# XiSHEN0220/RANSAC-Flow

Measured on AMD Instinct MI355X. Metric: aligned image-pairs/sec @480×640, 1/2/4/8 MI355X; max-abs flow Δ vs ref, higher is better.
Workload: dtype f32

## Files before the change

include/rfx_api.h:

```cpp
#ifndef RFX_API_H
#define RFX_API_H

#include <stddef.h>
#include <stdint.h>

#ifdef __cplusplus
extern "C" {
#endif

#define RFX_OK 0
#define RFX_E_ARG (-1)
#define RFX_E_LIMIT (-2)

#define RFX_ACT_NONE 0
#define RFX_ACT_RELU 1
#define RFX_ACT_SIGMOID 2

const char* rfx_version(void);

#define RFX_ABI_VERSION 12
int rfx_abi_version(void);

int rfx_group_begin(void);
int rfx_group_end(void* stream);
int rfx_group_abort(void);
int rfx_group_side_streams(int enable);

int rfx_conv2d_f32(const float* in, const float* wT, const int32_t* ktab, const float* scale,
                   const float* shift, const float* residual, float* out, int N, int Cin, int Hin,
                   int Win, int Cout, int KH, int KW, int stride, int pad, int act, void* stream);

int rfx_conv2d_tile_variant(int N, int Cout, int Hout, int Wout);

int rfx_conv2d_kernel_id(int N, int Cin, int Cout, int KH, int KW, int stride, int pad, int Hout, int Wout);

int rfx_conv3x3_f32(const float* in, const float* wP, const float* scale, const float* shift, const float* residual,
                    float* out, int N, int Cin, int H, int W, int Cout, int act, int k_chunk, void* stream);
int rfx_conv3x3_kernel_id(int N, int Cin, int Cout, int H, int W, int k_chunk);
int rfx_conv3x3_s2_f32(const float* in, const float* wP, const float* scale, const float* shift, const float* residual,
                       float* out, int N, int Cin, int H, int W, int Cout, int act, void* stream);

int rfx_conv3x3_conv1x1_kernel_id(int N, int H, int W, int Cmid);
int rfx_conv3x3_conv1x1_f32(const float* in, const float* wP2, const float* scale2, const float* shift2, int act2,
                            const float* wQ3, const float* scale3, const float* shift3, const float* residual, int act3,
                            float* out, int N, int Cin, int H, int W, int Cmid, int Cexp, void* stream);

int rfx_maxpool2d_f32(const float* in, float* out, int NC, int Hin, int Win, int k, int stride,
                      int pad, void* stream);

int rfx_blurpool2d_f32(const float* in, float* out, int NC, int Hin, int Win, int stride, void* stream);

int rfx_maxblurpool2d_f32(const float* in, float* out, int NC, int Hin, int Win, int stride, void* stream);

int rfx_stem_conv3x3_maxblur_f32(const float* in, const float* wT, const float* scale, const float* shift, float* out,
                                 int N, int H, int W, int Cout, void* stream);

int rfx_stem_conv7x7_maxpool_f32(const float* in, const float* wT, const float* scale, const float* shift, float* out,
                                 int N, int H, int W, int Cout, void* stream);

int rfx_l2norm_nchw_f32(const float* in, float* out, int N, int C, int HW, long long out_batch_stride,
                        long long out_chan_stride, void* stream);
int rfx_l2norm_nchw_scatter_f32(const float* in, float* out, int N, int C, int HW, const long long* dst_off,
                                long long out_chan_stride, void* stream);

int rfx_flow_head_f32(const float* logits, float* flow, int N, int K, int rows, int cols, void* stream);

int rfx_resize_bilinear_f32(const float* in, float* out, int NC, int Hin, int Win, int Hout, int Wout,
                            int align_corners, void* stream);

int rfx_lanczos_pass_u8(const uint8_t* in, uint8_t* out, int N, int inH, int inW, int outH, int outW, int C,
                        const int32_t* bounds, const int32_t* weights, int ksize, int vertical, int row_offset,
                        void* stream);

int rfx_u8_to_f32_chw(const uint8_t* in, float* raw, float* norm, int N, int H, int W, const float* mean3_host,
                      const float* std3_host, void* stream);

int rfx_copy_cols_f32(const float* src, float* dst, long long rows, int w_src, int w_dst, void* stream);

int rfx_corr_neigh_f32(const float* x, const float* y, float* out, int N, int C, int H, int W, int K,
                       void* stream);
int rfx_corr_neigh_variant_f32(const float* x, const float* y, float* out, int N, int C, int H, int W, int K,
                               int variant, void* stream);

int rfx_corr_neigh_bidir_f32(const float* x, const float* y, float* out_xy, float* out_yx, int N, int C, int H, int W, int K,
                             void* stream);
int rfx_corr_timing(int enable);
int rfx_corr_timing_collect(float* us_out, int cap);

int rfx_warp_grid_f32(const float* Hm, float* grid, int B, int h, int w, void* stream);

int rfx_grid_sample_f32(const float* in, const float* grid, float* out, int N, int C, int Hi, int Wi,
                        int Ho, int Wo, int align_corners, void* stream);

int rfx_compose_flow_f32(const float* flowDown, const float* coarseGrid, float* flow12, float* inb,
                         float* flowUp, int N, int hd, int wd, int Hc, int Wc, int H, int W, int clamp, void* stream);

int rfx_flow_grad_clamp_f32(const float* flowCoarse, const float* grid, float* flowGrad, float* flow, int B, int H, int W,
                            int grid_batch, void* stream);

int rfx_merge_multi_h_f32(const float* flow, const float* match12, long long match12_stride, const float* cyc,
                          const float* inb, int n, long long HW, float th, int multiH, float* flowGlobal,
                          float* matchGlobal, uint8_t* binary, void* stream);

int rfx_match_score_f32(const float* match12, long long match12_stride, const float* cyc, const float* inb, int n,
                        long long HW, float* score, void* stream);

size_t rfx_remove_small_cc_ws_bytes(int N, int H, int W);
int rfx_remove_small_cc_f32(const float* in, float* out, int N, int H, int W, float match_th, int max_area, void* ws,
                            void* stream);

size_t rfx_mutual_nn_ws_bytes(int nA, int nB);
int rfx_mutual_nn_f32(const float* featA, int ldA, int nA, const float* featB, int ldB, int nB, int C,
                      const float* maskB, int64_t* idx1, int64_t* idx2, int32_t* count, void* ws, int score_chunk,
                      void* stream);

int rfx_mutual_nn_batched_f32(const float* featA, int ldA, int nA, long long strideA, const float* featB, int ldB,
                              int nB, long long strideB, int C, const float* maskB, int64_t* idx1, int64_t* idx2,
                              int32_t* count, void* ws, int batch, int score_chunk, void* stream);

int rfx_mutual_nn_ragged_f32(const float* featA, int ldA, const float* featB, int ldB, const int32_t* nA, const int32_t* nB,
                             int maxNA, int maxNB, int C, const float* maskB, int64_t* idx1, int64_t* idx2, int cap,
                             int32_t* count, void* ws, int batch, int score_chunk, void* stream);

int rfx_dlt4_homography(const float* X, const float* Y, int N, float* Hout, void* stream);

int rfx_prediction_f32(const float* match1, const float* match2, int n, const float* Hs, int N, float* err,
                       void* stream);

int rfx_score_hypotheses(const float* match1, const float* match2, int n, const int64_t* samples, int N,
                         float tol, float* Hout, int64_t* counts, uint8_t* flags_out, void* ws, void* stream);

size_t rfx_ransac_ws_bytes(int n, int N);
int rfx_ransac_h4(const float* match1, const float* match2, int n, const int64_t* samples, int N,
                  float tol, float* bestH, uint8_t* inlier, int32_t* result, void* ws, void* stream);

size_t rfx_ransac_batched_ws_bytes(int cap, int N, int batch);
int rfx_ransac_h4_batched(const float* match1, const float* match2, const int32_t* n, int cap, const int64_t* samples,
                          int N, float tol, float* bestH, uint8_t* inlier, int32_t* result, void* ws, int batch,
                          void* stream);

int rfx_ransac_h4_batched_stage(const float* match1, const float* match2, const int32_t* n, int cap, const int64_t* samples,
                                int N, float tol, float* bestH, uint8_t* inlier, int32_t* result, void* ws, int batch,
                                int stages, void* stream);
int rfx_ransac_degenerate_list(const void* ws, int cap, int N, int batch, int32_t* idx, int32_t* count, int kcap, void* stream);
int rfx_ransac_patch_h(void* ws, int cap, int N, int batch, const int32_t* idx, const int32_t* count, const float* Hpatch,
                       int kcap, void* stream);
int rfx_ransac_degenerate_gather(const void* ws, const float* match1, const float* match2, const int32_t* n, int cap,
                                 const int64_t* samples, int N, int batch, int32_t* idx, int32_t* count, int32_t* off,
                                 int32_t* off_host, float* xy_rows, int row_cap, void* stream);
int rfx_ransac_patch_h_rows(void* ws, int cap, int N, int batch, const int32_t* idx, const int32_t* count, const int32_t* off,
                            const float* H_rows, int row_cap, void* stream);
int rfx_dlt4_homography_flags(const float* X, const float* Y, int N, float* Hout, uint8_t* flags, void* stream);

int rfx_gather_matches_f32(const int64_t* idx1, const int64_t* idx2, const int32_t* n, int cap, const float* xa,
                           const float* ya, const float* xb, const float* yb, float* match1, float* match2, int batch,
                           void* stream);

int rfx_gather_matches_ragged_f32(const int64_t* idx1, const int64_t* idx2, const int32_t* n, int cap, const float* xa,
                                  const float* ya, const long long* offA, const float* xb, const float* yb, const long long* offB,
                                  float* match1, float* match2, int batch, void* stream);

int rfx_draw_samples_i64(const int32_t* n, int64_t* samples, int N, int batch, uint64_t seed, uint64_t stream_id,
                         const int32_t* pair_ids, void* stream);

int rfx_keep_mask_f32(const float* mask, const float* bg, const int32_t* active, int n_active, int h, int w, int rt, int ct,
                      float* keep, void* stream);

int rfx_filter_matches_f32(const int64_t* idx1, const int64_t* idx2, const int32_t* count, int cap, const int32_t* active,
                           int n_active, const float* mask, const float* bg, int h, int w, int rt, int ct, const float* xa,
                           const float* ya, const float* xb, const float* yb, float* match1, float* match2, int32_t* n_out,
                           int32_t* kept, void* stream);

size_t rfx_multih_accept_ws_bytes(int n_active);
int rfx_multih_accept_f32(const float* match, float* mask, const float* bg, const int32_t* active, int n_active, int h, int w,
                          const int32_t* ransac_result, const int32_t* n_match, int32_t* nbH, double th, int mode,
                          int32_t* accept, float* gain, void* ws, const float* bestH, const float* flowDown8,
                          const float* match12Down8, const float* match21Down8, int h8, int w8, const float* flowD2, int hd2,
                          int wd2, float* rec, long long rec_stride, int max_h, int off_H, int off_flow, int off_match,
                          int off_d2, void* stream);

int rfx_filter_matches_ragged_f32(const int64_t* idx1, const int64_t* idx2, const int32_t* count, int cap, const int32_t* active,
                                  int n_active, const float* mask, const float* bg, const long long* moff, const int32_t* geom,
                                  const float* xa, const float* ya, const long long* offA, const float* xb, const float* yb,
                                  const long long* offB, float* match1, float* match2, int32_t* n_out, int32_t* kept,
                                  void* stream);

size_t rfx_multih_accept_ragged_ws_bytes(int n_active);
int rfx_multih_accept_ragged_f32(const float* match, const long long* match_off, float* mask, const float* bg,
                                 const long long* moff, const int32_t* geom, const int32_t* active, int n_active, long long max_hw,
                                 const int32_t* ransac_result, const int32_t* n_match, int32_t* nbH, double th, int mode,
                                 int32_t* accept, float* gain, void* ws, const float* bestH, const float* flowDown8,
                                 const float* match12Down8, const float* match21Down8, const long long* off8, float* rec,
                                 long long rec_stride, int max_h, int off_H, int off_flow, void* stream);

int rfx_conv1x1_split_f32(const float* in, const void* wS, const float* scale, const float* shift, const float* residual,
                          float* out, int N, int Cin, int HW, int Cout, int act, void* stream);
int rfx_conv1x1_split_strided_f32(const float* in, const void* wS, const float* scale, const float* shift, const float* residual,
                                  float* out, int N, int Cin, int Hin, int Win, int Cout, int stride, int act, void* stream);
int rfx_conv3x3_split_f32(const float* in, const void* wS3, const float* scale, const float* shift, const float* residual,
                          float* out, int N, int Cin, int H, int W, int Cout, int act, void* stream);
int rfx_conv3x3_split_s2_f32(const float* in, const void* wS3, const float* scale, const float* shift, const float* residual,
                             float* out, int N, int Cin, int H, int W, int Cout, int act, void* stream);

int rfx_conv2d_dilated_f32(const float* in, const float* wT, const int32_t* ktab, const float* scale,
                           const float* shift, const float* residual, float* out, int N, int Cin, int Hin,
                           int Win, int Cout, int KH, int KW, int stride, int pad, int dilation, int act, void* stream);
int rfx_adaptive_avgpool2d_f32(const float* in, float* out, int NC, int Hin, int Win, int Hout, int Wout, void* stream);
int rfx_softmax_accum_f32(const float* logits, float* scores, int N, int C, long long HW, float div, int accumulate, void* stream);
int rfx_argmax_mask_f32(const float* scores, int N, int C, long long HW, int id, int complement, float* mask, int32_t* pred,
                        void* stream);

#ifdef __cplusplus
}
#endif
#endif
```

ransac-flow_amd/csrc/conv1x1s.hip:

```cpp
#include "common.h"
#include "conv_epilogue.h"
#include "group.h"

namespace {

typedef __bf16 bf16x8 __attribute__((ext_vector_type(8)));
typedef __bf16 bf16x2 __attribute__((ext_vector_type(2)));
typedef float f32x2 __attribute__((ext_vector_type(2)));
typedef unsigned u32x4 __attribute__((ext_vector_type(4)));

struct C1SArgs {
    const float* in; const u32x4* wS; const float* scale; const float* shift; const float* res; float* out;
    int Cin, HW, Cout, act, Mpad;
    long long P;
    int tilesM, tilesP;
    int stride, Win, Wo, HWin;
};

__device__ __forceinline__ unsigned pack_bf16(float a, float b) {
    const f32x2 v = {a, b};
    const bf16x2 h = __builtin_convertvector(v, bf16x2);
    unsigned u;
    __builtin_memcpy(&u, &h, 4);
    return u;
}
__device__ __forceinline__ void split_pair(float a, float b, unsigned& hi, unsigned& mid, unsigned& lo) {
    hi = pack_bf16(a, b);
    const float ra = a - __uint_as_float(hi << 16), rb = b - __uint_as_float(hi & 0xffff0000u);
    mid = pack_bf16(ra, rb);
    lo = pack_bf16(ra - __uint_as_float(mid << 16), rb - __uint_as_float(mid & 0xffff0000u));
}
__device__ __forceinline__ bf16x8 as_frag(const u32x4& w) {
    bf16x8 f;
    __builtin_memcpy(&f, &w, 16);
    return f;
}

template <int TM>
__device__ __forceinline__ void conv1x1_split_body(const C1SArgs& a, const unsigned bx) {
    constexpr int BM = 64 * TM, BN = 128, KB = 16;
    constexpr int A_WORDS = 3 * 2 * BM;
    constexpr int NA = (A_WORDS + 255) / 256;
    __shared__ u32x4 As[2][3][2][BM];
    __shared__ u32x4 Bs[2][3][2][BN];
    __shared__ float s_scale[BM], s_shift[BM];

    const int t = threadIdx.x, lane = t & 63, wave = t >> 6;
    const int wm = wave >> 1, wn = wave & 1;
    const int lrow = lane >> 5, lcol = lane & 31;
    const size_t HW = (size_t)a.HW, HWin = (size_t)a.HWin;
    const int nwg = a.tilesM * a.tilesP;
    const int nk = a.Cin / KB;

    int m0; long long n0;
    {
        const int v = (int)bx, q = nwg / 8, r = nwg % 8, xcd = v % 8, j = v / 8;
        const int bid = (xcd < r ? xcd * (q + 1) : r * (q + 1) + (xcd - r) * q) + j;
        m0 = (bid % a.tilesM) * BM;
        n0 = (long long)(bid / a.tilesM) * BN;
    }
    constexpr int A_ROWS = 256 / BM;
    const u32x4* wsrc = a.wS + (size_t)(t / BM) * a.Mpad + m0 + t % BM;
    auto a_on = [&](int j) { return (j + 1) * 256 <= A_WORDS || t + 256 * j < A_WORDS; };
    const int bh = t >> 7, bp = t & 127;
    const float* bsrc;
    {
        long long p = n0 + bp;
        if (p >= a.P) p = a.P - 1;
        const long long n = p / a.HW;
        int off = (int)(p - n * a.HW);
        if (a.stride != 1) { const int y = off / a.Wo, x = off - y * a.Wo; off = y * a.stride * a.Win + x * a.stride; }
        bsrc = a.in + ((size_t)n * a.Cin + 8 * bh) * HWin + (size_t)off;
    }
    u32x4 ra[NA];
    float rb[8];
    auto load_stage = [&](int kb) {
#pragma unroll
        for (int j = 0; j < NA; ++j)
            ra[j] = wsrc[((size_t)kb * 6 + (a_on(j) ? A_ROWS * j : 0)) * a.Mpad];
#pragma unroll
        for (int i = 0; i < 8; ++i) rb[i] = bsrc[(size_t)(kb * KB + i) * HWin];
    };
    auto store_stage = [&](int buf) {
#pragma unroll
        for (int j = 0; j < NA; ++j)
            if (a_on(j)) (&As[buf][0][0][0])[t + 256 * j] = ra[j];
        u32x4 hi, mid, lo;
#pragma unroll
        for (int i = 0; i < 4; ++i) {
            unsigned h_, m_, l_;
            split_pair(rb[2 * i], rb[2 * i + 1], h_, m_, l_);
            hi[i] = h_; mid[i] = m_; lo[i] = l_;
        }
        Bs[buf][0][bh][bp] = hi;
        Bs[buf][1][bh][bp] = mid;
        Bs[buf][2][bh][bp] = lo;
    };
    if (t < BM) {
        const int m = m0 + t;
        s_scale[t] = (a.scale && m < a.Cout) ? a.scale[m] : 1.0f;
        s_shift[t] = (a.shift && m < a.Cout) ? a.shift[m] : 0.0f;
    }
    load_stage(0);
    store_stage(0);
    if (nk > 1) load_stage(1);
    __syncthreads();

    f32x16 acc[TM][2], low[TM][2];
#pragma unroll
    for (int i = 0; i < TM; ++i)
#pragma unroll
        for (int j = 0; j < 2; ++j)
#pragma unroll
            for (int r = 0; r < 16; ++r) { acc[i][j][r] = 0.0f; low[i][j][r] = 0.0f; }

    for (int s = 0; s < nk; ++s) {
        const int cur = s & 1;
        bf16x8 af[3][TM], bf[3][2];
#pragma unroll
        for (int pc = 0; pc < 3; ++pc) {
#pragma unroll
            for (int i = 0; i < TM; ++i) af[pc][i] = as_frag(As[cur][pc][lrow][wm * TM * 32 + i * 32 + lcol]);
#pragma unroll
            for (int j = 0; j < 2; ++j) bf[pc][j] = as_frag(Bs[cur][pc][lrow][wn * 64 + j * 32 + lcol]);
        }
        if (s + 1 < nk) store_stage(cur ^ 1);
        if (s + 2 < nk) load_stage(s + 2);
        __builtin_amdgcn_sched_barrier(0);
#pragma unroll
        for (int i = 0; i < TM; ++i)
#pragma unroll
            for (int j = 0; j < 2; ++j) {
                low[i][j] = __builtin_amdgcn_mfma_f32_32x32x16_bf16(af[2][i], bf[0][j], low[i][j], 0, 0, 0);
                low[i][j] = __builtin_amdgcn_mfma_f32_32x32x16_bf16(af[0][i], bf[2][j], low[i][j], 0, 0, 0);
                low[i][j] = __builtin_amdgcn_mfma_f32_32x32x16_bf16(af[1][i], bf[1][j], low[i][j], 0, 0, 0);
            }
#pragma unroll
        for (int i = 0; i < TM; ++i)
#pragma unroll
            for (int j = 0; j < 2; ++j) {
                low[i][j] = __builtin_amdgcn_mfma_f32_32x32x16_bf16(af[1][i], bf[0][j], low[i][j], 0, 0, 0);
                low[i][j] = __builtin_amdgcn_mfma_f32_32x32x16_bf16(af[0][i], bf[1][j], low[i][j], 0, 0, 0);
                acc[i][j] = __builtin_amdgcn_mfma_f32_32x32x16_bf16(af[0][i], bf[0][j], acc[i][j], 0, 0, 0);
            }
        __builtin_amdgcn_sched_barrier(0);
        __syncthreads();
    }
#pragma unroll
    for (int i = 0; i < TM; ++i)
#pragma unroll
        for (int j = 0; j < 2; ++j)
#pragma unroll
            for (int r = 0; r < 16; ++r) acc[i][j][r] += low[i][j][r];

    size_t pix_off[2];
    bool pix_ok[2];
#pragma unroll
    for (int j = 0; j < 2; ++j) {
        long long pp = n0 + wn * 64 + j * 32 + lcol;
        pix_ok[j] = pp < a.P;
        if (!pix_ok[j]) pp = a.P - 1;
        const long long n = pp / a.HW;
        pix_off[j] = (size_t)n * a.Cout * HW + (size_t)(pp - n * a.HW);
    }
    conv_epilogue<TM, 2, false>(acc, s_scale, s_shift, a.res, a.out, a.act, a.Cout, HW, m0, wm, lrow, pix_off, pix_ok, m0 + BM <= a.Cout);
}

template <int TM>
__global__ __launch_bounds__(256, 2) void conv1x1_split_kernel(C1SArgs a) {
    conv1x1_split_body<TM>(a, blockIdx.x);
}

template <int TM>
__global__ __launch_bounds__(256, 2) void conv1x1_split_group_kernel(RfxGroupArgs<C1SArgs> g) {
    const unsigned y = blockIdx.y;
    if (blockIdx.x >= g.gx[y]) return;
    conv1x1_split_body<TM>(g.p[y], blockIdx.x);
}

template <int TM>
static int c1s_group_launch(const void* blob, const unsigned* gx, int n, hipStream_t st) {
    return rfx_group_launch_impl<C1SArgs>(conv1x1_split_group_kernel<TM>, 256, blob, gx, n, st);
}

template <int TM>
int launch_split(C1SArgs& a, hipStream_t st) {
    a.tilesM = (a.Cout + 64 * TM - 1) / (64 * TM);
    a.tilesP = (int)((a.P + 127) / 128);
    const long long nwg = (long long)a.tilesM * a.tilesP;
    if (nwg > 0x7fffffffLL) return RFX_E_LIMIT;
    if (rfx_group_recording()) return rfx_group_record(&c1s_group_launch<TM>, &a, sizeof(a), (unsigned)nwg);
    hipLaunchKernelGGL((conv1x1_split_kernel<TM>), dim3((unsigned)nwg), dim3(256), 0, st, a);
    RFX_LAUNCH_CHECK();
    return RFX_OK;
}

}

static int conv1x1_split_launch(const float* in, const void* wS, const float* scale, const float* shift, const float* residual,
                                float* out, int N, int Cin, int Hin, int Win, int Cout, int stride, int act, void* stream) {
    if (!in || !wS || !out || N <= 0 || Cin <= 0 || Hin <= 0 || Win <= 0 || Cout <= 0) return RFX_E_ARG;
    if (Cin % 16 != 0 || (stride != 1 && stride != 2)) return RFX_E_ARG;
    if (act != RFX_ACT_NONE && act != RFX_ACT_RELU && act != RFX_ACT_SIGMOID) return RFX_E_ARG;
    const int Ho = (Hin - 1) / stride + 1, Wo = (Win - 1) / stride + 1;
    C1SArgs a;
    a.in = in; a.wS = reinterpret_cast<const u32x4*>(wS); a.scale = scale; a.shift = shift; a.res = residual; a.out = out;
    a.Cin = Cin; a.HW = Ho * Wo; a.Cout = Cout; a.act = act; a.Mpad = (Cout + 127) / 128 * 128;
    a.P = (long long)N * a.HW;
    a.stride = stride; a.Win = Win; a.Wo = Wo; a.HWin = Hin * Win;
    return Cout > 64 ? launch_split<2>(a, rfx_stream(stream)) : launch_split<1>(a, rfx_stream(stream));
}

extern "C" int rfx_conv1x1_split_f32(const float* in, const void* wS, const float* scale, const float* shift, const float* residual,
                                     float* out, int N, int Cin, int HW, int Cout, int act, void* stream) {
    return conv1x1_split_launch(in, wS, scale, shift, residual, out, N, Cin, 1, HW, Cout, 1, act, stream);
}

extern "C" int rfx_conv1x1_split_strided_f32(const float* in, const void* wS, const float* scale, const float* shift, const float* residual,
                                             float* out, int N, int Cin, int Hin, int Win, int Cout, int stride, int act, void* stream) {
    return conv1x1_split_launch(in, wS, scale, shift, residual, out, N, Cin, Hin, Win, Cout, stride, act, stream);
}
```

ransac-flow_amd/rfx/_lib.py:

```python
import ctypes
import os
from ctypes import c_int, c_int32, c_int64, c_uint64, c_float, c_double, c_void_p, c_size_t, c_longlong, c_char_p

_HERE = os.path.dirname(os.path.abspath(__file__))
LIB_PATH = os.environ.get("RFX_LIB") or os.path.normpath(os.path.join(_HERE, "..", "librfx.so"))

SIGNATURES = {
    "rfx_version": (c_char_p, []),
    "rfx_abi_version": (c_int, []),
    "rfx_group_begin": (c_int, []),
    "rfx_group_end": (c_int, [c_void_p]),
    "rfx_group_abort": (c_int, []),
    "rfx_group_side_streams": (c_int, [c_int]),
    "rfx_conv2d_f32": (c_int, [c_void_p] * 7 + [c_int] * 10 + [c_void_p]),
    "rfx_conv2d_dilated_f32": (c_int, [c_void_p] * 7 + [c_int] * 11 + [c_void_p]),
    "rfx_conv1x1_split_f32": (c_int, [c_void_p] * 6 + [c_int] * 5 + [c_void_p]),
    "rfx_conv3x3_split_f32": (c_int, [c_void_p] * 6 + [c_int] * 6 + [c_void_p]),
    "rfx_conv3x3_split_s2_f32": (c_int, [c_void_p] * 6 + [c_int] * 6 + [c_void_p]),
    "rfx_conv1x1_split_strided_f32": (c_int, [c_void_p] * 6 + [c_int] * 7 + [c_void_p]),
    "rfx_adaptive_avgpool2d_f32": (c_int, [c_void_p, c_void_p] + [c_int] * 5 + [c_void_p]),
    "rfx_softmax_accum_f32": (c_int, [c_void_p, c_void_p, c_int, c_int, c_longlong, c_float, c_int, c_void_p]),
    "rfx_argmax_mask_f32": (c_int, [c_void_p, c_int, c_int, c_longlong, c_int, c_int, c_void_p, c_void_p, c_void_p]),
    "rfx_conv2d_tile_variant": (c_int, [c_int] * 4),
    "rfx_conv2d_kernel_id": (c_int, [c_int] * 9),
    "rfx_conv3x3_f32": (c_int, [c_void_p] * 6 + [c_int] * 7 + [c_void_p]),
    "rfx_conv3x3_kernel_id": (c_int, [c_int] * 6),
    "rfx_conv3x3_s2_f32": (c_int, [c_void_p] * 6 + [c_int] * 6 + [c_void_p]),
    "rfx_conv3x3_conv1x1_kernel_id": (c_int, [c_int] * 4),
    "rfx_conv3x3_conv1x1_f32": (c_int, [c_void_p] * 4 + [c_int] + [c_void_p] * 4 + [c_int, c_void_p] + [c_int] * 6 + [c_void_p]),
    "rfx_maxpool2d_f32": (c_int, [c_void_p, c_void_p] + [c_int] * 6 + [c_void_p]),
    "rfx_blurpool2d_f32": (c_int, [c_void_p, c_void_p] + [c_int] * 4 + [c_void_p]),
    "rfx_maxblurpool2d_f32": (c_int, [c_void_p, c_void_p] + [c_int] * 4 + [c_void_p]),
    "rfx_stem_conv3x3_maxblur_f32": (c_int, [c_void_p] * 5 + [c_int] * 4 + [c_void_p]),
    "rfx_stem_conv7x7_maxpool_f32": (c_int, [c_void_p] * 5 + [c_int] * 4 + [c_void_p]),
    "rfx_l2norm_nchw_f32": (c_int, [c_void_p, c_void_p, c_int, c_int, c_int, c_longlong, c_longlong, c_void_p]),
    "rfx_l2norm_nchw_scatter_f32": (c_int, [c_void_p, c_void_p, c_int, c_int, c_int, c_void_p, c_longlong, c_void_p]),
    "rfx_flow_head_f32": (c_int, [c_void_p, c_void_p] + [c_int] * 4 + [c_void_p]),
    "rfx_resize_bilinear_f32": (c_int, [c_void_p, c_void_p] + [c_int] * 6 + [c_void_p]),
    "rfx_lanczos_pass_u8": (c_int, [c_void_p, c_void_p] + [c_int] * 6 + [c_void_p, c_void_p] + [c_int] * 3 + [c_void_p]),
    "rfx_u8_to_f32_chw": (c_int, [c_void_p] * 3 + [c_int] * 3 + [c_void_p] * 3),
    "rfx_copy_cols_f32": (c_int, [c_void_p, c_void_p, c_longlong, c_int, c_int, c_void_p]),
    "rfx_corr_neigh_f32": (c_int, [c_void_p] * 3 + [c_int] * 5 + [c_void_p]),
    "rfx_corr_neigh_variant_f32": (c_int, [c_void_p] * 3 + [c_int] * 6 + [c_void_p]),
    "rfx_corr_neigh_bidir_f32": (c_int, [c_void_p] * 4 + [c_int] * 5 + [c_void_p]),
    "rfx_corr_timing": (c_int, [c_int]),
    "rfx_corr_timing_collect": (c_int, [c_void_p, c_int]),
    "rfx_warp_grid_f32": (c_int, [c_void_p, c_void_p] + [c_int] * 3 + [c_void_p]),
    "rfx_grid_sample_f32": (c_int, [c_void_p] * 3 + [c_int] * 7 + [c_void_p]),
    "rfx_compose_flow_f32": (c_int, [c_void_p] * 5 + [c_int] * 8 + [c_void_p]),
    "rfx_flow_grad_clamp_f32": (c_int, [c_void_p] * 4 + [c_int] * 4 + [c_void_p]),
    "rfx_merge_multi_h_f32": (c_int, [c_void_p, c_void_p, c_longlong, c_void_p, c_void_p, c_int, c_longlong, c_float, c_int,
                                      c_void_p, c_void_p, c_void_p, c_void_p]),
    "rfx_match_score_f32": (c_int, [c_void_p, c_longlong, c_void_p, c_void_p, c_int, c_longlong, c_void_p, c_void_p]),
    "rfx_remove_small_cc_ws_bytes": (c_size_t, [c_int] * 3),
    "rfx_remove_small_cc_f32": (c_int, [c_void_p, c_void_p, c_int, c_int, c_int, c_float, c_int, c_void_p, c_void_p]),
    "rfx_mutual_nn_ws_bytes": (c_size_t, [c_int, c_int]),
    "rfx_mutual_nn_f32": (c_int, [c_void_p, c_int, c_int, c_void_p, c_int, c_int, c_int] + [c_void_p] * 5 + [c_int, c_void_p]),
    "rfx_mutual_nn_batched_f32": (c_int, [c_void_p, c_int, c_int, c_longlong, c_void_p, c_int, c_int, c_longlong, c_int]
                                  + [c_void_p] * 5 + [c_int, c_int, c_void_p]),
    "rfx_mutual_nn_ragged_f32": (c_int, [c_void_p, c_int, c_void_p, c_int, c_void_p, c_void_p, c_int, c_int, c_int, c_void_p,
                                         c_void_p, c_void_p, c_int, c_void_p, c_void_p, c_int, c_int, c_void_p]),
    "rfx_dlt4_homography": (c_int, [c_void_p, c_void_p, c_int, c_void_p, c_void_p]),
    "rfx_prediction_f32": (c_int, [c_void_p, c_void_p, c_int, c_void_p, c_int, c_void_p, c_void_p]),
    "rfx_score_hypotheses": (c_int, [c_void_p, c_void_p, c_int, c_void_p, c_int, c_float] + [c_void_p] * 5),
    "rfx_ransac_ws_bytes": (c_size_t, [c_int, c_int]),
    "rfx_ransac_h4": (c_int, [c_void_p, c_void_p, c_int, c_void_p, c_int, c_float] + [c_void_p] * 5),
    "rfx_ransac_batched_ws_bytes": (c_size_t, [c_int, c_int, c_int]),
    "rfx_ransac_h4_batched_stage": (c_int, [c_void_p, c_void_p, c_void_p, c_int, c_void_p, c_int, c_float] + [c_void_p] * 4
                                    + [c_int, c_int, c_void_p]),
    "rfx_ransac_degenerate_list": (c_int, [c_void_p, c_int, c_int, c_int, c_void_p, c_void_p, c_int, c_void_p]),
    "rfx_ransac_patch_h": (c_int, [c_void_p, c_int, c_int, c_int, c_void_p, c_void_p, c_void_p, c_int, c_void_p]),
    "rfx_ransac_degenerate_gather": (c_int, [c_void_p] * 4 + [c_int, c_void_p, c_int, c_int] + [c_void_p] * 5 + [c_int, c_void_p]),
    "rfx_ransac_patch_h_rows": (c_int, [c_void_p, c_int, c_int, c_int] + [c_void_p] * 4 + [c_int, c_void_p]),
    "rfx_dlt4_homography_flags": (c_int, [c_void_p, c_void_p, c_int, c_void_p, c_void_p, c_void_p]),
    "rfx_ransac_h4_batched": (c_int, [c_void_p, c_void_p, c_void_p, c_int, c_void_p, c_int, c_float] + [c_void_p] * 4
                              + [c_int, c_void_p]),
    "rfx_gather_matches_f32": (c_int, [c_void_p, c_void_p, c_void_p, c_int] + [c_void_p] * 6 + [c_int, c_void_p]),
    "rfx_gather_matches_ragged_f32": (c_int, [c_void_p, c_void_p, c_void_p, c_int] + [c_void_p] * 8 + [c_int, c_void_p]),
    "rfx_draw_samples_i64": (c_int, [c_void_p, c_void_p, c_int, c_int, c_uint64, c_uint64, c_void_p, c_void_p]),
    "rfx_filter_matches_f32": (c_int, [c_void_p, c_void_p, c_void_p, c_int, c_void_p, c_int, c_void_p, c_void_p] + [c_int] * 4
                               + [c_void_p] * 9),
    "rfx_keep_mask_f32": (c_int, [c_void_p] * 3 + [c_int] * 5 + [c_void_p, c_void_p]),
    "rfx_multih_accept_ws_bytes": (c_size_t, [c_int]),
    "rfx_multih_accept_f32": (c_int, [c_void_p] * 4 + [c_int] * 3 + [c_void_p] * 3 + [c_double, c_int] + [c_void_p] * 7
                              + [c_int, c_int, c_void_p, c_int, c_int, c_void_p, c_longlong] + [c_int] * 5 + [c_void_p]),
    "rfx_filter_matches_ragged_f32": (c_int, [c_void_p, c_void_p, c_void_p, c_int, c_void_p, c_int] + [c_void_p] * 15),
    "rfx_multih_accept_ragged_ws_bytes": (c_size_t, [c_int]),
    "rfx_multih_accept_ragged_f32": (c_int, [c_void_p] * 7 + [c_int, c_longlong] + [c_void_p] * 3 + [c_double, c_int]
                                     + [c_void_p] * 9 + [c_longlong] + [c_int] * 3 + [c_void_p]),
}

ABI_VERSION = 12

_lib = None


def load():
    global _lib
    if _lib is not None:
        return _lib
    import torch
    if not os.path.exists(LIB_PATH):
        raise RuntimeError(
            "librfx.so not found at %s -- build it with `python -c 'import __graft_entry__ as g; g.build()'` "
            "(hipcc --offload-arch=gfx950).  There is no CPU fallback." % LIB_PATH)
    lib = ctypes.CDLL(LIB_PATH)
    for name, (res, args) in SIGNATURES.items():
        try:
            fn = getattr(lib, name)
        except AttributeError as e:
            raise RuntimeError("librfx.so is missing symbol %s (stale build?)" % name) from e
        fn.restype = res
        fn.argtypes = args
    if lib.rfx_abi_version() != ABI_VERSION:
        raise RuntimeError("librfx.so has ABI revision %d, this binding was written against %d (stale build?): rebuild with "
                           "`make -C ransac-flow_amd/csrc`" % (lib.rfx_abi_version(), ABI_VERSION))
    _lib = lib
    return lib


class RfxError(RuntimeError):
    pass


def check(rc, what):
    if rc != 0:
        kind = "bad argument" if rc == -1 else ("limit exceeded" if rc == -2 else "hipError_t %d" % rc)
        raise RfxError("%s failed: %s" % (what, kind))
```

Before: 160.7.

## Add wide 256-channel 512-thread tile variant for split-bf16 1x1 conv

Adds a 512-thread, 8-wave variant of the split-precision 1x1 conv kernel covering 256 output channels per workgroup, so each staged input tile is reused across twice as many output channels. A heuristic picks the wide tile for large Cout/Cin layers when a wave-count cost model over the CU count predicts fewer effective waves than the 128-channel tile. The B-stage load is split across twice as many threads with 2-element packing. It trades occupancy (one block per CU, larger LDS) for less redundant activation loading and splitting.

```diff
diff --git a/include/rfx_api.h b/include/rfx_api.h
--- a/include/rfx_api.h
+++ b/include/rfx_api.h
@@ -18,7 +18,7 @@
 
 const char* rfx_version(void);
 
-#define RFX_ABI_VERSION 12
+#define RFX_ABI_VERSION 13
 int rfx_abi_version(void);
 
 int rfx_group_begin(void);
@@ -197,6 +197,7 @@
                           float* out, int N, int Cin, int HW, int Cout, int act, void* stream);
 int rfx_conv1x1_split_strided_f32(const float* in, const void* wS, const float* scale, const float* shift, const float* residual,
                                   float* out, int N, int Cin, int Hin, int Win, int Cout, int stride, int act, void* stream);
+int rfx_conv1x1_split_tile_channels(int N, int Cin, int HWout, int Cout);
 int rfx_conv3x3_split_f32(const float* in, const void* wS3, const float* scale, const float* shift, const float* residual,
                           float* out, int N, int Cin, int H, int W, int Cout, int act, void* stream);
 int rfx_conv3x3_split_s2_f32(const float* in, const void* wS3, const float* scale, const float* shift, const float* residual,
diff --git a/ransac-flow_amd/csrc/conv1x1s.hip b/ransac-flow_amd/csrc/conv1x1s.hip
--- a/ransac-flow_amd/csrc/conv1x1s.hip
+++ b/ransac-flow_amd/csrc/conv1x1s.hip
@@ -8,6 +8,7 @@
 typedef __bf16 bf16x2 __attribute__((ext_vector_type(2)));
 typedef float f32x2 __attribute__((ext_vector_type(2)));
 typedef unsigned u32x4 __attribute__((ext_vector_type(4)));
+typedef unsigned u32x2 __attribute__((ext_vector_type(2)));
 
 struct C1SArgs {
     const float* in; const u32x4* wS; const float* scale; const float* shift; const float* res; float* out;
@@ -36,11 +37,12 @@
     return f;
 }
 
-template <int TM>
+template <int TM, int WM>
 __device__ __forceinline__ void conv1x1_split_body(const C1SArgs& a, const unsigned bx) {
-    constexpr int BM = 64 * TM, BN = 128, KB = 16;
+    constexpr int BM = 32 * TM * WM, BN = 128, KB = 16, NT = 128 * WM;
     constexpr int A_WORDS = 3 * 2 * BM;
-    constexpr int NA = (A_WORDS + 255) / 256;
+    constexpr int NA = (A_WORDS + NT - 1) / NT;
+    constexpr bool WIDE = WM == 4;
     __shared__ u32x4 As[2][3][2][BM];
     __shared__ u32x4 Bs[2][3][2][BN];
     __shared__ float s_scale[BM], s_shift[BM];
@@ -59,9 +61,11 @@
         m0 = (bid % a.tilesM) * BM;
         n0 = (long long)(bid / a.tilesM) * BN;
     }
-    constexpr int A_ROWS = 256 / BM;
+    constexpr int A_ROWS = NT / BM;
     const u32x4* wsrc = a.wS + (size_t)(t / BM) * a.Mpad + m0 + t % BM;
-    auto a_on = [&](int j) { return (j + 1) * 256 <= A_WORDS || t + 256 * j < A_WORDS; };
+    if (WIDE && m0 + t % BM >= a.Mpad) wsrc = a.wS + (size_t)(t / BM) * a.Mpad + a.Mpad - 1;
+    auto a_on = [&](int j) { return (j + 1) * NT <= A_WORDS || t + NT * j < A_WORDS; };
+    constexpr int NB = 2048 / NT;
     const int bh = t >> 7, bp = t & 127;
     const float* bsrc;
     {
@@ -70,31 +74,45 @@
         const long long n = p / a.HW;
         int off = (int)(p - n * a.HW);
         if (a.stride != 1) { const int y = off / a.Wo, x = off - y * a.Wo; off = y * a.stride * a.Win + x * a.stride; }
-        bsrc = a.in + ((size_t)n * a.Cin + 8 * bh) * HWin + (size_t)off;
+        bsrc = a.in + ((size_t)n * a.Cin + NB * bh) * HWin + (size_t)off;
     }
     u32x4 ra[NA];
-    float rb[8];
+    float rb[NB];
     auto load_stage = [&](int kb) {
 #pragma unroll
         for (int j = 0; j < NA; ++j)
             ra[j] = wsrc[((size_t)kb * 6 + (a_on(j) ? A_ROWS * j : 0)) * a.Mpad];
 #pragma unroll
-        for (int i = 0; i < 8; ++i) rb[i] = bsrc[(size_t)(kb * KB + i) * HWin];
+        for (int i = 0; i < NB; ++i) rb[i] = bsrc[(size_t)(kb * KB + i) * HWin];
     };
     auto store_stage = [&](int buf) {
 #pragma unroll
         for (int j = 0; j < NA; ++j)
-            if (a_on(j)) (&As[buf][0][0][0])[t + 256 * j] = ra[j];
-        u32x4 hi, mid, lo;
-#pragma unroll
-        for (int i = 0; i < 4; ++i) {
-            unsigned h_, m_, l_;
-            split_pair(rb[2 * i], rb[2 * i + 1], h_, m_, l_);
-            hi[i] = h_; mid[i] = m_; lo[i] = l_;
+            if (a_on(j)) (&As[buf][0][0][0])[t + NT * j] = ra[j];
+        if constexpr (NB == 8) {
+            u32x4 hi, mid, lo;
+#pragma unroll
+            for (int i = 0; i < 4; ++i) {
+                unsigned h_, m_, l_;
+                split_pair(rb[2 * i], rb[2 * i + 1], h_, m_, l_);
+                hi[i] = h_; mid[i] = m_; lo[i] = l_;
+            }
+            Bs[buf][0][bh][bp] = hi;
+            Bs[buf][1][bh][bp] = mid;
+            Bs[buf][2][bh][bp] = lo;
+        } else {
+            u32x2 hi, mid, lo;
+#pragma unroll
+            for (int i = 0; i < 2; ++i) {
+                unsigned h_, m_, l_;
+                split_pair(rb[2 * i], rb[2 * i + 1], h_, m_, l_);
+                hi[i] = h_; mid[i] = m_; lo[i] = l_;
+            }
+            u32x2* w = reinterpret_cast<u32x2*>(&Bs[buf][0][bh >> 1][bp]) + (bh & 1);
+            w[0] = hi;
+            w[4 * BN] = mid;
+            w[8 * BN] = lo;
         }
-        Bs[buf][0][bh][bp] = hi;
-        Bs[buf][1][bh][bp] = mid;
-        Bs[buf][2][bh][bp] = lo;
     };
     if (t < BM) {
         const int m = m0 + t;
@@ -168,14 +186,24 @@
 
 template <int TM>
 __global__ __launch_bounds__(256, 2) void conv1x1_split_kernel(C1SArgs a) {
-    conv1x1_split_body<TM>(a, blockIdx.x);
+    conv1x1_split_body<TM, 2>(a, blockIdx.x);
 }
 
 template <int TM>
 __global__ __launch_bounds__(256, 2) void conv1x1_split_group_kernel(RfxGroupArgs<C1SArgs> g) {
     const unsigned y = blockIdx.y;
     if (blockIdx.x >= g.gx[y]) return;
-    conv1x1_split_body<TM>(g.p[y], blockIdx.x);
+    conv1x1_split_body<TM, 2>(g.p[y], blockIdx.x);
+}
+
+__global__ __launch_bounds__(512, 1) void conv1x1_split_wide_kernel(C1SArgs a) {
+    conv1x1_split_body<2, 4>(a, blockIdx.x);
+}
+
+__global__ __launch_bounds__(512, 1) void conv1x1_split_wide_group_kernel(RfxGroupArgs<C1SArgs> g) {
+    const unsigned y = blockIdx.y;
+    if (blockIdx.x >= g.gx[y]) return;
+    conv1x1_split_body<2, 4>(g.p[y], blockIdx.x);
 }
 
 template <int TM>
@@ -183,14 +211,41 @@
     return rfx_group_launch_impl<C1SArgs>(conv1x1_split_group_kernel<TM>, 256, blob, gx, n, st);
 }
 
-template <int TM>
+static int c1s_wide_group_launch(const void* blob, const unsigned* gx, int n, hipStream_t st) {
+    return rfx_group_launch_impl<C1SArgs>(conv1x1_split_wide_group_kernel, 512, blob, gx, n, st);
+}
+
+int c1s_tile_channels(long long P, int Cin, int Cout) {
+    static const int mode = [] { const char* e = getenv("RFX_C1S_WIDE"); return e ? (atoi(e) == 0 ? 0 : 1) : -1; }();
+    static const long long cus = [] {
+        int dev = 0, n = 256;
+        if (hipGetDevice(&dev) == hipSuccess) hipDeviceGetAttribute(&n, hipDeviceAttributeMultiprocessorCount, dev);
+        return (long long)(n > 0 ? n : 256);
+    }();
+    if (Cout <= 64) return 64;
+    if (Cout < 256 || mode == 0) return 128;
+    if (mode == 1) return 256;
+    if (Cin < 512) return 128;
+    const long long tp = (P + 127) / 128, w = (Cout + 255) / 256 * tp, n = (Cout + 127) / 128 * tp;
+    const long long rest = n % (2 * cus);
+    const long long cost_wide = (w + cus - 1) / cus * 81, cost_128 = n / (2 * cus) * 100 + (rest == 0 ? 0 : rest <= cus ? 58 : 100);
+    return cost_wide < cost_128 ? 256 : 128;
+}
+
+template <int TM, int WM>
 int launch_split(C1SArgs& a, hipStream_t st) {
-    a.tilesM = (a.Cout + 64 * TM - 1) / (64 * TM);
+    constexpr int BM = 32 * TM * WM;
+    a.tilesM = (a.Cout + BM - 1) / BM;
     a.tilesP = (int)((a.P + 127) / 128);
     const long long nwg = (long long)a.tilesM * a.tilesP;
     if (nwg > 0x7fffffffLL) return RFX_E_LIMIT;
-    if (rfx_group_recording()) return rfx_group_record(&c1s_group_launch<TM>, &a, sizeof(a), (unsigned)nwg);
-    hipLaunchKernelGGL((conv1x1_split_kernel<TM>), dim3((unsigned)nwg), dim3(256), 0, st, a);
+    if constexpr (WM == 4) {
+        if (rfx_group_recording()) return rfx_group_record(&c1s_wide_group_launch, &a, sizeof(a), (unsigned)nwg);
+        hipLaunchKernelGGL(conv1x1_split_wide_kernel, dim3((unsigned)nwg), dim3(512), 0, st, a);
+    } else {
+        if (rfx_group_recording()) return rfx_group_record(&c1s_group_launch<TM>, &a, sizeof(a), (unsigned)nwg);
+        hipLaunchKernelGGL((conv1x1_split_kernel<TM>), dim3((unsigned)nwg), dim3(256), 0, st, a);
+    }
     RFX_LAUNCH_CHECK();
     return RFX_OK;
 }
@@ -208,7 +263,16 @@
     a.Cin = Cin; a.HW = Ho * Wo; a.Cout = Cout; a.act = act; a.Mpad = (Cout + 127) / 128 * 128;
     a.P = (long long)N * a.HW;
     a.stride = stride; a.Win = Win; a.Wo = Wo; a.HWin = Hin * Win;
-    return Cout > 64 ? launch_split<2>(a, rfx_stream(stream)) : launch_split<1>(a, rfx_stream(stream));
+    switch (c1s_tile_channels(a.P, Cin, Cout)) {
+        case 256: return launch_split<2, 4>(a, rfx_stream(stream));
+        case 128: return launch_split<2, 2>(a, rfx_stream(stream));
+        default: return launch_split<1, 2>(a, rfx_stream(stream));
+    }
+}
+
+extern "C" int rfx_conv1x1_split_tile_channels(int N, int Cin, int HWout, int Cout) {
+    if (N <= 0 || Cin <= 0 || HWout <= 0 || Cout <= 0) return RFX_E_ARG;
+    return c1s_tile_channels((long long)N * HWout, Cin, Cout);
 }
 
 extern "C" int rfx_conv1x1_split_f32(const float* in, const void* wS, const float* scale, const float* shift, const float* residual,
diff --git a/ransac-flow_amd/rfx/_lib.py b/ransac-flow_amd/rfx/_lib.py
--- a/ransac-flow_amd/rfx/_lib.py
+++ b/ransac-flow_amd/rfx/_lib.py
@@ -18,6 +18,7 @@
     "rfx_conv3x3_split_f32": (c_int, [c_void_p] * 6 + [c_int] * 6 + [c_void_p]),
     "rfx_conv3x3_split_s2_f32": (c_int, [c_void_p] * 6 + [c_int] * 6 + [c_void_p]),
     "rfx_conv1x1_split_strided_f32": (c_int, [c_void_p] * 6 + [c_int] * 7 + [c_void_p]),
+    "rfx_conv1x1_split_tile_channels": (c_int, [c_int] * 4),
     "rfx_adaptive_avgpool2d_f32": (c_int, [c_void_p, c_void_p] + [c_int] * 5 + [c_void_p]),
     "rfx_softmax_accum_f32": (c_int, [c_void_p, c_void_p, c_int, c_int, c_longlong, c_float, c_int, c_void_p]),
     "rfx_argmax_mask_f32": (c_int, [c_void_p, c_int, c_int, c_longlong, c_int, c_int, c_void_p, c_void_p, c_void_p]),
@@ -90,7 +91,7 @@
                                      + [c_void_p] * 9 + [c_longlong] + [c_int] * 3 + [c_void_p]),
 }
 
-ABI_VERSION = 12
+ABI_VERSION = 13
 
 _lib = None
 
```

After: 162.4 (median of 6 runs). 1.0% higher.
